# NYXFLOWER/GripNet

Measured on AMD Instinct MI355X. Metric: edges aggregated/sec, GripNet forward on pose-0, higher is better.
Workload: dtype f32

## Files before the change

### gripnet_amd/_hip.py

```python
from __future__ import annotations

import ctypes as C
import operator
import os
import threading

import torch

from ._cache import MISS, VersionedCache

_LIB_PATH = os.environ.get("GN_HIP_LIBRARY") or os.path.join(os.path.dirname(os.path.abspath(__file__)), "lib",
                                                            "libgripnet_hip.so")
_lib = None
_lock = threading.Lock()

GN_OK, GN_ERR_INVALID_ARG, GN_ERR_HIP, GN_ERR_INDEX_RANGE, GN_ERR_UNSUPPORTED, GN_ERR_EDGE_COUNT = range(6)
GN_RGCN_PARTIAL, GN_RGCN_ARITH_FAST, GN_RGCN_BASIS_TRANSPOSED = 1, 4, 64
GN_RGCN_PATH_SHIFT = 8
RGCN_PATHS = {"auto": 0, "pair": 1, "lds": 3, "general": 4, "table": 5}
GN_GEMM_RELU, GN_GEMM_ARITH_FAST, GN_GEMM_B_TRANSPOSED, GN_GEMM_ACCUMULATE, GN_GEMM_A_TRANSPOSED, GN_GEMM_JOIN_BATCH, GN_GEMM_OUT_BF16 = 1, 2, 4, 8, 16, 32, 64
GN_DM_TYPES_SORTED = 1
GN_DM_TYPE_TASKS = 2
ABI_VERSION = 162

_p, _i64, _int, _sz = C.c_void_p, C.c_int64, C.c_int, C.c_size_t

SIGNATURES = {
    "gn_version": (_int, []),
    "gn_last_error": (C.c_char_p, []),
    "gn_time_next_launch": (_int, [_p, _p]),
    "gn_host_scratch_release": (_sz, []),
    "gn_device_blocks_live": (_i64, []),
    "gn_time_launch_pending": (_int, []),
    "gn_gcn_plan_create": (_int, [_p, _p, _p, _i64, _i64, _int, _p, C.POINTER(_p)]),
    "gn_bipartite_plan_create": (_int, [_p, _p, _p, _i64, _i64, _i64, _p, C.POINTER(_p)]),
    "gn_sum_plan_create": (_int, [_p, _p, _p, _i64, _i64, _i64, _p, C.POINTER(_p)]),
    "gn_graph_plan_destroy": (None, [_p]),
    "gn_graph_plan_input_edges": (_i64, [_p]),
    "gn_graph_plan_nnz": (_i64, [_p]),
    "gn_graph_plan_export": (_int, [_p, _p, _p, _p]),
    "gn_graph_aggregate_f32": (_int, [_p, _p, _i64, _i64, _p, _i64, _p, _int, _p, _i64, _p, _p, _p]),
    "gn_split_planes_bytes": (_sz, [_i64, _int]),
    "gn_split_planes_f32": (_int, [_p, _i64, _i64, _i64, _i64, _p, _p]),
    "gn_transform_fusable": (_int, [_i64, _i64]),
    "gn_graph_transform_fusable": (_int, [_p, _i64, _i64]),
    "gn_graph_plan_build_blocked": (_int, [_p, _i64, _p]),
    "gn_graph_plan_blocked_cols": (_i64, [_p]),
    "gn_graph_blocked_applicable": (_int, [_p, _p, _i64, _i64, _p, _i64, _p, _p, _i64]),
    "gn_graph_chain_applicable": (_int, [_p, _p, _p, _i64, _i64, _p, _i64, _p, _p, _i64, _p]),
    "gn_graph_aggregate_chain_f32": (_int, [_p, _p, _p, _i64, _i64, _p, _i64, _p, _int, _p, _i64, _p, _p]),
    "gn_graph_gather_chained_f32": (_int, [_p, _p, _i64, _p]),
    "gn_graph_aggregate_tail_f32": (_int, [_p, _p, _i64, _i64, _p, _i64, _p, _int, _p, _i64, _p, _p, _p, _p, _int, _p]),
    "gn_graph_plan_build_transpose": (_int, [_p, _p]),
    "gn_graph_aggregate_t_f32": (_int, [_p, _p, _i64, _i64, _p, _i64, _p]),
    "gn_xtg_wide_supported": (_int, [_i64, _i64, _i64]),
    "gn_gemm_f32": (_int, [_p, _i64, _i64, _p, _i64, _p, _i64, _i64, _p, _i64, _i64, _i64, _i64, _i64, _i64, _p, _int, _p]),
    "gn_gemm_addend_f32": (_int, [_p, _i64, _i64, _p, _i64, _p, _i64, _i64, _p, _i64, _i64, _i64, _i64, _i64, _i64, _p, _p, _i64, _int, _p]),
    "gn_merge_f32": (_int, [_p, _i64, _p, _i64, _p, _i64, _i64, _i64, _int, _p]),
    "gn_softmax_rows_f32": (_int, [_p, _i64, _i64, _i64, _p]),
    "gn_softmax_rows_backward_f32": (_int, [_p, _i64, _p, _i64, _p, _i64, _i64, _i64, _p]),
    "gn_class_scores_f32": (_int, [_p, _i64, _i64, _p, _i64, _p, _i64, _i64, _i64, _int, _p, _i64, _p]),
    "gn_rgcn_plan_create": (_int, [_p, _p, _p, _int, _i64, _i64, _i64, _i64, _i64, _p, C.POINTER(_p)]),
    "gn_rgcn_plan_create_ex": (_int, [_p, _p, _p, _int, _i64, _i64, _i64, _i64, _i64, _int, _p, C.POINTER(_p)]),
    "gn_rgcn_plan_destroy": (None, [_p]),
    "gn_rgcn_plan_input_edges": (_i64, [_p]),
    "gn_rgcn_workspace_bytes": (_sz, [_p, _i64, _i64, _i64, _int]),
    "gn_rgcn_forward_path": (_int, [_p, _i64, _i64, _i64, _int]),
    "gn_rgcn_forward_choice": (_int, [_p, _p, _i64, _i64, _i64, _i64, _int, C.POINTER(_sz)]),
    "gn_cast_bf16": (_int, [_p, _i64, _p, _i64, _i64, _i64, _p]),
    "gn_graph_aggregate_bf16": (_int, [_p, _p, _i64, _i64, _p, _int, _p, _i64, _p, _p]),
    "gn_rgcn_forward_f32": (_int, [_p, _p, _i64, _i64, _p, _p, _i64, _p, _p, _i64, _int, _int, _p, _i64, _p, _p, _p, _sz, _p]),
    "gn_rgcn_finalize_f32": (_int, [_p, _p, _i64, _p, _i64, _i64, _p, _p, _i64, _int, _p, _i64, _p, _p]),
    "gn_distmult_forward_f32": (_int, [_p, _i64, _i64, _i64, _p, _p, _p, _p, _i64, _i64, _i64, _int, _p, _p, _p]),
    "gn_distmult_packed_forward_f32": (_int, [_p, _i64, _i64, _i64, _p, _p, _p, _i64, _i64, _i64, _int, _p, _p, _p]),
    "gn_distmult_plan_create": (_int, [_p, _p, _p, _i64, _i64, _i64, _i64, _p, C.POINTER(_p)]),
    "gn_distmult_plan_destroy": (None, [_p]),
    "gn_distmult_plan_edges": (_i64, [_p]),
    "gn_distmult_plan_forward_f32": (_int, [_p, _p, _i64, _i64, _p, _i64, _int, _p, _p]),
    "gn_distmult_plan_forward_cols_f32": (_int, [_p, _p, _i64, _i64, _i64, _i64, _p, _i64, _int, _p, _p]),
    "gn_xtg_workspace_bytes": (_sz, [_i64, _i64]),
# ... 223 lines not shown
    def __init__(self):
        self.calls, self.keep = [], []

    def __enter__(self):
        global _recorder
        self._prev, _recorder = _recorder, self
        return self

    def __exit__(self, *exc):
        global _recorder
        _recorder = self._prev


_recorder = None


def replay(calls):
    t = _timer
    for fn, args, name, tag in calls:
        if t is not None and (t.only is None or name in t.only):
            seen = t._seen.get(name, 0)
            t._seen[name] = seen + 1
            if seen % t.every == 0:
                status = _timed_call(t, fn, args, name, tag)
                if status:
                    check(status)
                continue
        status = fn(*args)
        if status:
            check(status)


_ENV_HOOKS = ("GN_DISABLE_FAST", "GN_DISABLE_QUAD", "GN_DISABLE_BLOCKED", "GN_BLOCKED_ANY", "GN_DISABLE_LDS_TABLE",
              "GN_ENABLE_CHAIN")
_ENV_NEUTRAL = ("GN_PLAN_THREADS", "GN_SAMPLER_TASKS", "GN_RGCN_SLAB_MB")
_ENV_DATA = getattr(os.environ, "_data", None)
_ENV_KEYS = tuple(k.encode() for k in _ENV_HOOKS) if isinstance(_ENV_DATA, dict) and all(isinstance(k, bytes) for k in list(_ENV_DATA)[:1]) else None


def release_host_scratch() -> int:
    return int(load().gn_host_scratch_release())


def device_blocks_live() -> int:
    return int(load().gn_device_blocks_live())


def env_stamp():
    if _ENV_KEYS is not None:
        d = _ENV_DATA
        return tuple([d.get(k) for k in _ENV_KEYS])
    return tuple([os.environ.get(k) for k in _ENV_HOOKS])


def launch_context(device):
    index = device.index
    return torch.cuda.current_device(), (_raw_stream(index) if _raw_stream is not None else torch.cuda.current_stream(index).cuda_stream)


class CallMemo:

    DEPTH = 8

    def __init__(self):
        self.entries = {}
        self.last = None

# ... 257 lines not shown
        require_gpu(edge_index, edge_weight)
        ei, src, dst, e = edge_rows(edge_index)
        w = None if edge_weight is None else edge_weight.to(torch.float32).contiguous()
        if w is not None and w.numel() != e:
            raise ValueError("edge_weight has {} entries for {} edges".format(w.numel(), e))
        plan = cls(None, ei.device, kind)
        plan._create(create, ei.device, src, dst, ptr(w), e, int(size_a), int(size_b))
        plan.n_rows, plan.n_table = int(n_rows), int(n_table)
        return plan

    @classmethod
    def gcn(cls, edge_index, num_nodes, edge_weight=None, improved=False):
        return cls._build("gcn", "gn_gcn_plan_create", edge_index, edge_weight, num_nodes, num_nodes, num_nodes, bool(improved))

    @classmethod
    def bipartite(cls, edge_index, num_sources, num_targets, edge_weight=None):
        return cls._build("bipartite", "gn_bipartite_plan_create", edge_index, edge_weight, num_sources, num_targets,
                          num_sources, num_targets)

    @classmethod
    def plain_sum(cls, edge_index, num_sources, num_targets):
        return cls._build("sum", "gn_sum_plan_create", edge_index, None, num_sources, num_targets, num_sources, num_targets)

    def build_blocked(self, cols: int):
        if self.kind == "gcn" and cols <= 32:
            with torch.cuda.device(self.device):
                check(load().gn_graph_plan_build_blocked(self._h, 16 if cols <= 16 else 32, stream_ptr(self.device)))
        return self.blocked_cols

    @property
    def blocked_cols(self) -> int:
        return int(load().gn_graph_plan_blocked_cols(self._h))

    def blocked_ok(self, x: torch.Tensor, weight: torch.Tensor, bias, out: torch.Tensor) -> bool:
        return bool(load().gn_graph_blocked_applicable(self._h, x.data_ptr(), ld(x), x.shape[1], weight.data_ptr(), weight.shape[1],
                                                       None if bias is None else bias.data_ptr(), out.data_ptr(), ld(out)))

    def transform_ok(self, fin: int, fout: int, x: torch.Tensor) -> bool:
        return (bool(load().gn_graph_transform_fusable(self._h, int(fin), int(fout))) and ld(x) % 4 == 0
                and x.data_ptr() % 16 == 0)

    @property
    def input_edges(self) -> int:
        return int(load().gn_graph_plan_input_edges(self._h))

    @property
    def nnz(self) -> int:
        return int(load().gn_graph_plan_nnz(self._h))

    def export(self):
        if self._export is None:
            n = self.nnz
            ei = torch.empty((2, n), dtype=torch.int64, device=self.device)
            nrm = torch.empty((n,), dtype=torch.float32, device=self.device)
            check(load().gn_graph_plan_export(self._h, ptr(ei), ptr(nrm), stream_ptr(self.device)))
            self._export = (ei, nrm)
        return self._export

    def __iter__(self):
        return iter(self.export())

    def aggregate(self, xw: torch.Tensor, bias, relu: bool, out: torch.Tensor, side=None, weight=None, planes=None, tail=None):
        sc = side_copy(side)
        pd = None
        if planes is not None:
            pd = planes[0].desc(planes[1], planes[2])
# ... 653 lines not shown
```

### gripnet_amd/csrc/common.h

```cpp
#pragma once

#include <hip/hip_runtime.h>
#include <hip/hip_ext.h>

#include <algorithm>
#include <atomic>
#include <cstdarg>
#include <cstdint>
#include <cstdio>
#include <cstdlib>
#include <cstring>
#include <memory>
#include <thread>
#include <type_traits>
#include <vector>

#include "gripnet_hip.h"
#include "host_parallel.hpp"

namespace gn {

constexpr int kWave = 64;

inline char* error_buffer() {
// ... 166 lines not shown

struct LaunchEvents { hipEvent_t start = nullptr, stop = nullptr; };
LaunchEvents take_launch_events();

}

struct gn_graph_plan {
    int64_t input_edges = 0;
    int64_t nnz = 0;
    int64_t rows = 0;
    int64_t table_rows = 0;
    int64_t max_row_nnz = 0;
    int is_gcn = 0;
    gn::DevBuf<int32_t> rowptr;
    gn::DevBuf<int32_t> col;
    gn::DevBuf<float> coef;
    gn::DevBuf<int64_t> ref_edge_index;
    gn::DevBuf<float> ref_norm;
    int ell_ok = 0;
    gn::DevBuf<uint32_t> ell_col;
    gn::DevBuf<float> ell_coef;
    int has_transpose = 0;
    gn::DevBuf<int32_t> t_rowptr;
    gn::DevBuf<int32_t> t_col;
    gn::DevBuf<float> t_coef;
    gn::DevBuf<float> dis;
    int unit_weights = 0;
    int plain_ones = 0;
    int blk_ok = 0, blk_cols = 0;
    int blk_cw = 0;
    int blk_rows = 0;
    int blk_cells = 0;
    int64_t blk_iters = 0;
    gn::DevBuf<float> blk_dis;
    gn::DevBuf<int32_t> blk_tile_off;
    gn::DevBuf<int32_t> blk_tile_rows;
    gn::DevBuf<float> blk_tile_dis;
    gn::DevBuf<uint32_t> blk_ids;
    gn::DevBuf<int32_t> blk_cell;
    gn::DevBuf<float> blk_table;
};

struct gn_rgcn_plan {
    int64_t input_edges = 0;
    int64_t edge_lo = 0, edge_hi = 0;
    int64_t shard_edges = 0;
    int64_t num_nodes = 0;
    int64_t num_relations = 0;
    int64_t max_row_nnz = 0;
    gn::DevBuf<float> indeg;
    gn::DevBuf<int32_t> rowptr;
    gn::DevBuf<uint32_t> key;
    gn::DevBuf<int32_t> row_order;
    int64_t heavy_rows = 0;
    gn::DevBuf<int32_t> dw_items;
    int64_t n_dw_items = 0, n_dw_parts = 0;
    gn::DevBuf<int32_t> dw_multi;
    int64_t n_dw_multi = 0;
    gn::DevBuf<int32_t> seg_begin;
    gn::DevBuf<uint32_t> packed;
    gn::DevBuf<int32_t> wg_begin;
    gn::DevBuf<int32_t> wg_items;
    int fast_groups = 0, fast_ts = 0;
    size_t fast_lds_bytes = 0;
    int fast_cols = 32;
    int fast_ok = 0;
// ... 17 lines not shown
```

### gripnet_amd/csrc/distmult_quad.cuh

```cuda
#pragma once

#include "common.h"

namespace gn_dm {

constexpr int kMaxPhases = 8;
#ifndef GN_DM_THREADS
#define GN_DM_THREADS 1024
#endif
constexpr int kThreads = GN_DM_THREADS;
constexpr size_t kLdsBudget = 150 * 1024;

typedef float f32x2 __attribute__((ext_vector_type(2)));
typedef float f32x4 __attribute__((ext_vector_type(4)));


template <int CTRL>
__device__ __forceinline__ int dpp_i(int x) { return __builtin_amdgcn_mov_dpp(x, CTRL, 0xf, 0xf, true); }
template <int CTRL>
__device__ __forceinline__ float dpp_add(float x) {
    return x + __builtin_bit_cast(float, __builtin_amdgcn_update_dpp(0, __builtin_bit_cast(int, x), CTRL, 0xf, 0xf, false));
}
__device__ __forceinline__ float row_sum16(float x) {
    x = dpp_add<0xB1>(x);
    x = dpp_add<0x4E>(x);
    x = dpp_add<0x141>(x);
    x = dpp_add<0x140>(x);
    return x;
}

__device__ __forceinline__ float sigmoid_f32(float x) { return __builtin_amdgcn_rcpf(1.0f + __expf(-x)); }

template <int W4>
__device__ __forceinline__ void fill_table(float4* lds4, const float* __restrict__ z, int64_t ld_z, int n, int c0, int w4rt,
                                           int stride4, int tid) {
    const int w4 = W4 > 0 ? W4 : w4rt;
    const int total = n * w4;
    const int rot = (int)((blockIdx.x * 977u) % (unsigned)total);
    for (int base = 0; base < total; base += 8 * kThreads) {
        float4 v[8];
        int at[8];
#pragma unroll
        for (int k = 0; k < 8; ++k) {
            int i = min(base + k * kThreads + tid, total - 1) + rot;
            i = i < total ? i : i - total;
            const int row = i / w4, c4 = i - row * w4;
            at[k] = row * stride4 + c4;
            v[k] = *reinterpret_cast<const float4*>(z + (int64_t)row * ld_z + c0 + 4 * c4);
        }
#pragma unroll
        for (int k = 0; k < 8; ++k)
            if (base + k * kThreads + tid < total) lds4[at[k]] = v[k];
    }
    const int pad = stride4 - w4;
    for (int i = tid; i < n * pad; i += kThreads) {
// ... 71 lines not shown
```

### gripnet_amd/csrc/gcn_blocked.hip

```cpp
#include "aggregate.cuh"
#include "layout_blocked.hpp"

#include <algorithm>
#include <numeric>
#include <vector>

namespace {

typedef float f32x4 __attribute__((ext_vector_type(4)));
typedef uint32_t u32x2 __attribute__((ext_vector_type(2)));
typedef float f32x2 __attribute__((ext_vector_type(2)));

#ifndef GN_COL_THREADS
#define GN_COL_THREADS 1024
#endif
constexpr int kColThreads = GN_COL_THREADS;
constexpr int kColWaves = kColThreads / 64;
static_assert(kColWaves == gn_layout::kColLayoutWaves, "the plan cuts a range's tiles into the waves of one workgroup");
constexpr size_t kColLdsBytes = 160 * 1024;
constexpr int kColSlack = gn_layout::kColLayoutSlack;
constexpr int kWaveInts = 12;

bool blocked_disabled() {
    if (gn::fast_paths_disabled()) return true;
    const char* e = getenv("GN_DISABLE_BLOCKED");
    return e && e[0] == '1';
}

struct TransArgs {
    const float* x; int64_t ld_x;
    const float* w;
    const float* dis;
    float* table;
// ... 57 lines not shown
        for (int nt = 0; nt < NT; ++nt) {
            const f32x4 v = real ? acc[nt] * scale : (f32x4){0.f, 0.f, 0.f, 0.f};
            if constexpr (CW == 2) {
                float* o = a.table + ((size_t)(8 * nt + 2 * j) * a.rows_pad + row) * 2;
                *reinterpret_cast<f32x2*>(o) = (f32x2){v[0], v[1]};
                *reinterpret_cast<f32x2*>(o + (size_t)a.rows_pad * 2) = (f32x2){v[2], v[3]};
            } else {
                float* o = a.table + (size_t)(16 * nt + 4 * j) * a.rows_pad + row;
#pragma unroll
                for (int c = 0; c < 4; ++c) o[(size_t)c * a.rows_pad] = v[c];
            }
        }
    }
}

struct ColArgs {
    const float* table;
    const int32_t* cell;
    const int32_t* tile_off;
    const int32_t* tile_rows;
    const float* tile_dis;
    const u32x2* ids;
    const float* dis; const float* bias;
    float* out; int64_t ld_out;
    int n, rows_pad, groups, ranges, relu;
    gn_side_copy side;
    float* next_table;
};

#ifdef GN_STAMPS
__device__ unsigned long long g_blk_stamps[2][512][4];
#endif

template <int CW, bool NEXT>
__device__ __forceinline__ void col_gather(const ColArgs& a, int stamp_set) {
    typedef float vec_t __attribute__((ext_vector_type(CW)));
    extern __shared__ f32x4 lds4[];
    const int tid = threadIdx.x, lane = tid & 63;
    const int wave = __builtin_amdgcn_readfirstlane(tid >> 6);
    const int q = lane >> 2, j = lane & 3;
    const int wg = blockIdx.x, per_x = (a.ranges + 7) / 8;
    const int x = wg & 7, k = wg >> 3;
    const int range = x * per_x + k / a.groups, cg = k % a.groups;
    const bool live = range < a.ranges;
#ifdef GN_STAMPS
    const unsigned long long st0 = __builtin_amdgcn_s_memrealtime();
#endif
    const int32_t* __restrict__ cell = a.cell + ((size_t)(live ? range : 0) * kColWaves + wave) * kWaveInts;
    const int c0 = cell[0], c1 = cell[1];
    int it = cell[2];
    const int it_last = cell[3];
    const int e0 = cell[4], e1 = cell[5], e2 = cell[6], e3 = cell[7], e4 = cell[8];
    if (live) {
        const int total = a.rows_pad * CW / 4;
        const f32x4* __restrict__ src = reinterpret_cast<const f32x4*>(a.table + (size_t)cg * a.rows_pad * CW);
        for (int i = wave * 64; i < total; i += kColThreads)
            __builtin_amdgcn_global_load_lds((const __attribute__((address_space(1))) void*)(src + i + lane),
                                             (__attribute__((address_space(3))) void*)(lds4 + i), 16, 0, 0);
    }
    do {
    if (!live) break;
    asm volatile("" ::: "memory");
    int tile_end = e0;
    const u32x2* __restrict__ sp = a.ids + (size_t)it * 64 + lane;
    u32x2 wa[8], wb[8];
#pragma unroll
    for (int k = 0; k < 8; ++k) wa[k] = sp[64 * k];
#pragma unroll
    for (int k = 0; k < 8; ++k) wb[k] = sp[512 + 64 * k];
    sp += 1024;
    const int32_t* __restrict__ trp = a.tile_rows + (size_t)c0 * 16 + q;
    const float* __restrict__ tdp = a.tile_dis + (size_t)c0 * 16 + q;
    int row = trp[0];
    const int row1 = trp[16], row2 = trp[32], row3 = trp[48];
    float d = tdp[0];
    const float d1 = tdp[16], d2 = tdp[32], d3 = tdp[48];
    int t = c0;
    vec_t bias = (vec_t)(0.f);
    if (a.bias) bias = *reinterpret_cast<const vec_t*>(a.bias + CW * cg);
    asm volatile("s_waitcnt vmcnt(0)" ::: "memory");
    __syncthreads();
#ifdef GN_STAMPS
    const unsigned long long st1 = __builtin_amdgcn_s_memrealtime();
#endif
    const vec_t* __restrict__ tab = reinterpret_cast<const vec_t*>(lds4);
    vec_t acc = (vec_t)(0.f);
#define GN_COL_FLUSH()                                                                                         \
    do {                                                                                                       \
        _Pragma("unroll") for (int c = 0; c < CW; ++c) {                                                       \
            float v = acc[c];                                                                                  \
            v += __shfl_xor(v, 1);                                                                             \
            v += __shfl_xor(v, 2);                                                                             \
            acc[c] = v;                                                                                        \
        }                                                                                                      \
        if (j == 0 && row >= 0) {                                                                              \
            vec_t r = acc * d + bias;                                                                          \
            if (a.relu) {                                                                                      \
                _Pragma("unroll") for (int c = 0; c < CW; ++c) r[c] = fmaxf(r[c], 0.f);                        \
            }                                                                                                  \
            *reinterpret_cast<vec_t*>(a.out + (int64_t)row * a.ld_out + CW * cg) = r;                          \
            if constexpr (NEXT)                                                                                \
                *reinterpret_cast<vec_t*>(a.next_table + ((size_t)cg * a.rows_pad + row) * CW) = r * d;        \
        }                                                                                                      \
        acc = (vec_t)(0.f);                                                                                    \
        ++t;                                                                                                   \
        const int kk = t - c0;                                                                                 \
        tile_end = kk == 1 ? e1 : (kk == 2 ? e2 : (kk == 3 ? e3 : (kk == 4 ? e4 : a.tile_off[t + 1])));       \
        if (kk < 4) {                                                                                          \
            row = kk == 1 ? row1 : (kk == 2 ? row2 : row3);                                                    \
            d = kk == 1 ? d1 : (kk == 2 ? d2 : d3);                                                            \
        } else {                                                                                               \
            row = a.tile_rows[(size_t)t * 16 + q];                                                             \
            d = a.tile_dis[(size_t)t * 16 + q];                                                                \
        }                                                                                                      \
    } while (0)
#define GN_COL_CONSUME(w)                                                                                      \
    _Pragma("unroll") for (int k = 0; k < 8; ++k) {                                                            \
        while (t < c1 && it == tile_end) GN_COL_FLUSH();                                                       \
        if (it < it_last) {                                                                                    \
            const uint32_t s0 = w[k].x & 0xffffu, s1 = w[k].x >> 16, s2 = w[k].y & 0xffffu, s3 = w[k].y >> 16; \
            acc += (tab[s0] + tab[s1]) + (tab[s2] + tab[s3]);                                                  \
            ++it;                                                                                              \
        }                                                                                                      \
    }
    while (it < it_last) {
        GN_COL_CONSUME(wa)
        if (it >= it_last) break;
#pragma unroll
        for (int k = 0; k < 8; ++k) wa[k] = sp[64 * k];
        GN_COL_CONSUME(wb)
#pragma unroll
        for (int k = 0; k < 8; ++k) wb[k] = sp[512 + 64 * k];
        sp += 1024;
    }
    while (t < c1) GN_COL_FLUSH();
#undef GN_COL_CONSUME
#undef GN_COL_FLUSH
#ifdef GN_STAMPS
    if (tid == 0 && blockIdx.x < 512) {
        unsigned long long* o = g_blk_stamps[stamp_set & 1][blockIdx.x];
        o[0] = st0; o[1] = st1; o[2] = __builtin_amdgcn_s_memrealtime(); o[3] = 0;
    }
#endif
    } while (0);
    gn::side_copy_stream(a.side, blockIdx.x * (int64_t)blockDim.x + threadIdx.x, (int64_t)gridDim.x * blockDim.x);
}

template <int CW>
__global__ __launch_bounds__(kColThreads) void k_col_gather(ColArgs a, int stamp_set) { col_gather<CW, false>(a, stamp_set); }
template <int CW>
__global__ __launch_bounds__(kColThreads) void k_col_gather_next(ColArgs a, int stamp_set) { col_gather<CW, true>(a, stamp_set); }

template <int FIN, int NT>
void launch_transform(const TransArgs& t, int cw, hipStream_t st) {
    const int grid = (int)std::min<int64_t>(gn::ceil_div(t.rows_pad / 16, 4), GN_AGG_GRID);
    if (cw == 2) k_col_transform<FIN, NT, 2><<<grid, 256, 0, st>>>(t); else k_col_transform<FIN, NT, 1><<<grid, 256, 0, st>>>(t);
}

}

bool gn_blocked_applicable(const gn_graph_plan* plan, const float* x, int64_t ld_x, int64_t fin, const float* w, int64_t fout,
                           const float* bias, const float* out, int64_t ld_out) {
    if (!plan->blk_ok || blocked_disabled()) return false;
    const int cw = plan->blk_cw;
    if ((ld_out % cw) != 0 || (reinterpret_cast<uintptr_t>(out) % (4 * cw)) != 0 ||
        (bias && (reinterpret_cast<uintptr_t>(bias) % (4 * cw)) != 0)) return false;
    if (!(fout == 16 || fout == 32) || fout > plan->blk_cols) return false;
    if (w) {
        if (!(fin == 16 || fin == 32 || fin == 64)) return false;
        if (!gn::aligned16(w)) return false;
    } else if (fin != fout) {
        return false;
    }
    return (ld_x % 4) == 0 && gn::aligned16(x);
}

namespace {

gn_status blocked_transform(const gn_graph_plan* plan, const float* x, int64_t ld_x, int64_t fin, const float* w, int64_t fout,
                            hipStream_t st) {
    TransArgs t;
    t.x = x; t.ld_x = ld_x; t.w = w; t.dis = plan->blk_dis.p; t.table = plan->blk_table.p; t.n = (int)plan->rows;
    t.rows_pad = plan->blk_rows;
    const int cw = plan->blk_cw;
    switch ((int)((w ? fin : fout) * 100 + fout)) {
        case 1616: launch_transform<16, 1>(t, cw, st); break;
        case 3216: launch_transform<32, 1>(t, cw, st); break;
        case 6416: launch_transform<64, 1>(t, cw, st); break;
        case 1632: launch_transform<16, 2>(t, cw, st); break;
        case 3232: launch_transform<32, 2>(t, cw, st); break;
        case 6432: launch_transform<64, 2>(t, cw, st); break;
        default: return gn::fail(GN_ERR_UNSUPPORTED, "no LDS-staged kernel for %lld -> %lld features", (long long)fin, (long long)fout);
    }
    GN_LAUNCH_CHECK();
    return GN_OK;
}

gn_status blocked_gather(const gn_graph_plan* plan, int64_t fout, const float* bias, int relu, float* out, int64_t ld_out,
                         const gn_side_copy& side, float* next_table, int stamp_set, hipStream_t st) {
    const int cw = plan->blk_cw;
    GN_REQUIRE((ld_out % cw) == 0 && (reinterpret_cast<uintptr_t>(out) % (4 * cw)) == 0 &&
               (!bias || (reinterpret_cast<uintptr_t>(bias) % (4 * cw)) == 0),
               "the LDS-staged path writes %d-float column groups: out and bias must be aligned to them", cw);
    ColArgs a;
    a.table = plan->blk_table.p; a.cell = plan->blk_cell.p; a.tile_off = plan->blk_tile_off.p; a.tile_rows = plan->blk_tile_rows.p;
    a.tile_dis = plan->blk_tile_dis.p;
    a.ids = reinterpret_cast<const u32x2*>(plan->blk_ids.p); a.dis = plan->blk_dis.p; a.bias = bias;
    a.out = out; a.ld_out = ld_out; a.n = (int)plan->rows; a.rows_pad = plan->blk_rows;
    a.groups = (int)(fout / cw); a.ranges = plan->blk_cells; a.relu = relu; a.side = side; a.next_table = next_table;
    const int per_x = (a.ranges + 7) / 8;
    const int grid = 8 * per_x * a.groups;
    const size_t lds = (size_t)plan->blk_rows * cw * sizeof(float);
    auto launch = [&](auto kernel) {
        gn_status s = gn::allow_large_lds(reinterpret_cast<const void*>(kernel), (int)kColLdsBytes);
        if (s == GN_OK) kernel<<<grid, kColThreads, lds, st>>>(a, stamp_set);
        return s;
    };
    gn_status s;
    if (next_table) s = cw == 2 ? launch(k_col_gather_next<2>) : launch(k_col_gather_next<1>);
    else s = cw == 2 ? launch(k_col_gather<2>) : launch(k_col_gather<1>);
    if (s != GN_OK) return s;
    GN_LAUNCH_CHECK();
    return GN_OK;
}

bool chain_disabled() {
    const char* e = getenv("GN_ENABLE_CHAIN");
    return !(e && e[0] == '1') || blocked_disabled();
}

bool chain_plans_match(const gn_graph_plan* plan, const gn_graph_plan* next) {
    return plan && next && plan != next && plan->blk_ok && next->blk_ok && plan->is_gcn && next->is_gcn && plan->unit_weights &&
           next->unit_weights && plan->rows == next->rows && plan->nnz == next->nnz && plan->blk_rows == next->blk_rows &&
           plan->blk_cw == next->blk_cw && plan->blk_cells == next->blk_cells && plan->blk_iters == next->blk_iters &&
           next->blk_cols >= 16;
}

}

gn_status gn_blocked_aggregate(const gn_graph_plan* plan, const float* x, int64_t ld_x, int64_t fin, const float* w,
                               int64_t fout, const float* bias, int relu, float* out, int64_t ld_out,
                               const gn_side_copy& side, hipStream_t st) {
    const gn_status s = blocked_transform(plan, x, ld_x, fin, w, fout, st);
    return s != GN_OK ? s : blocked_gather(plan, fout, bias, relu, out, ld_out, side, nullptr, fin == 32 ? 0 : 1, st);
}

extern "C" int gn_graph_chain_applicable(const gn_graph_plan* plan, const gn_graph_plan* next, const float* x, int64_t ld_x,
                                         int64_t num_features, const float* weight, int64_t out_features, const float* bias,
                                         const float* out, int64_t ld_out, const float* out_next) {
    if (chain_disabled() || !chain_plans_match(plan, next) || !weight || out_features != 16) return 0;
    if (!gn_blocked_applicable(plan, x, ld_x, num_features, weight, out_features, bias, out, ld_out)) return 0;
    return (reinterpret_cast<uintptr_t>(out_next) % (4 * next->blk_cw)) == 0 ? 1 : 0;
}
// ... 46 lines not shown
        rows_pad = gn::ceil_div((N + 1) * cw * 4, 1024) * 1024 / (cw * 4);
        if (rows_pad * cw * 4 > (int64_t)kColLdsBytes) return GN_OK;
    }
    const int groups = (int)(cols / cw);
    const int R = std::max(1, std::min<int>(256 / groups, (int)gn::ceil_div(N, 64)));

    GN_LAP(nullptr);
    gn::ArenaHold arena;
    std::vector<int32_t> rp(N + 1), col(nnz);
    GN_HIP(hipMemcpyAsync(rp.data(), plan->rowptr.p, (N + 1) * sizeof(int32_t), hipMemcpyDeviceToHost, st));
    GN_HIP(hipMemcpyAsync(col.data(), plan->col.p, nnz * sizeof(int32_t), hipMemcpyDeviceToHost, st));
    std::vector<float> dis_host((size_t)rows_pad + 16, 0.f);
    GN_HIP(hipMemcpyAsync(dis_host.data(), plan->dis.p, N * sizeof(float), hipMemcpyDeviceToHost, st));
    GN_HIP(hipStreamSynchronize(st));

    GN_LAP("blocked: CSR to the host");
    gn_layout::BlockedLayout bl = gn_layout::build_blocked_layout(N, R, rp, col, dis_host);
    GN_LAP("blocked: host schedule");
    if (bl.failed) return gn::fail(GN_ERR_UNSUPPORTED, "internal: an edge was not scheduled");
    if (!bl.ok) return GN_OK;
    plan->blk_ok = 0;
    GN_HIP(plan->blk_dis.upload(dis_host, st));
    GN_HIP(plan->blk_tile_off.upload(bl.tile_off, st));
    GN_HIP(plan->blk_tile_rows.upload(bl.tile_rows, st));
    GN_HIP(plan->blk_tile_dis.upload(bl.tile_dis, st));
    GN_HIP(plan->blk_ids.upload(bl.ids.data(), bl.ids.size() / 2, st));
    GN_HIP(plan->blk_cell.upload(bl.cell, st));
    GN_HIP(plan->blk_table.alloc((size_t)rows_pad * cols));
    GN_HIP(hipMemsetAsync(plan->blk_table.p, 0, (size_t)rows_pad * cols * sizeof(float), st));
    GN_HIP(hipStreamSynchronize(st));
    GN_LAP("blocked: upload");
    plan->blk_cols = (int)cols; plan->blk_cw = cw; plan->blk_rows = (int)rows_pad; plan->blk_cells = R;
    plan->blk_iters = bl.iters_total;
    plan->blk_ok = 1;
    return GN_OK;
}

#ifdef GN_STAMPS
extern "C" __attribute__((visibility("default"))) int gn_debug_read_blk_stamps(unsigned long long* host_out) {
    return (int)hipMemcpyFromSymbol(host_out, HIP_SYMBOL(g_blk_stamps), sizeof(unsigned long long) * 2 * 512 * 4);
}
#endif

extern "C" int64_t gn_graph_plan_blocked_cols(const gn_graph_plan* plan) {
    return (plan && plan->blk_ok && !blocked_disabled()) ? plan->blk_cols : 0;
}
```

### include/gripnet_hip.h

```cpp
#ifndef GRIPNET_HIP_H
#define GRIPNET_HIP_H

#include <stddef.h>
#include <stdint.h>

#ifdef __cplusplus
extern "C" {
#endif

#define GN_VERSION 162

#if defined(GN_BUILDING)
#define GN_API __attribute__((visibility("default")))
#else
#define GN_API
#endif

typedef enum gn_status {
    GN_OK = 0,
    GN_ERR_INVALID_ARG = 1,
    GN_ERR_HIP = 2,
    GN_ERR_INDEX_RANGE = 3,
    GN_ERR_UNSUPPORTED = 4,
    GN_ERR_EDGE_COUNT = 5
} gn_status;

typedef struct gn_side_copy {
    const float* src; int64_t ld_src;
    float* dst; int64_t ld_dst;
    int64_t rows, cols;
    int mode;
} gn_side_copy;

typedef struct gn_split_planes {
    void* planes;
    int64_t rows;
    int nt;
    int col_main;
    int col_side;
} gn_split_planes;

typedef struct gn_graph_plan gn_graph_plan;
typedef struct gn_rgcn_plan gn_rgcn_plan;

GN_API int gn_version(void);
GN_API const char* gn_last_error(void);
GN_API int64_t gn_device_blocks_live(void);

GN_API gn_status gn_gcn_plan_create(const int64_t* src, const int64_t* dst, const float* w, int64_t num_edges,
                             int64_t num_nodes, int improved, void* stream, gn_graph_plan** plan);

GN_API gn_status gn_bipartite_plan_create(const int64_t* src, const int64_t* dst, const float* w, int64_t num_edges,
                                   int64_t num_sources, int64_t num_targets, void* stream, gn_graph_plan** plan);

GN_API gn_status gn_sum_plan_create(const int64_t* src, const int64_t* dst, const float* w, int64_t num_edges,
                             int64_t num_sources, int64_t num_targets, void* stream, gn_graph_plan** plan);

GN_API void gn_graph_plan_destroy(gn_graph_plan* plan);
GN_API int64_t gn_graph_plan_input_edges(const gn_graph_plan* plan);
GN_API int64_t gn_graph_plan_nnz(const gn_graph_plan* plan);
GN_API gn_status gn_graph_plan_export(const gn_graph_plan* plan, int64_t* edge_index_out, float* norm_out, void* stream);

GN_API gn_status gn_graph_aggregate_f32(const gn_graph_plan* plan, const float* xw, int64_t ld_xw, int64_t num_features,
                                 const float* weight , int64_t out_features,
                                 const float* bias, int relu, float* out, int64_t ld_out,
                                 const gn_side_copy* side , const gn_split_planes* planes ,
                                 void* stream);
GN_API size_t gn_split_planes_bytes(int64_t rows, int nt);
GN_API gn_status gn_split_planes_f32(const float* src, int64_t ld_src, int64_t rows, int64_t cols, int64_t col0,
                              const gn_split_planes* planes, void* stream);
GN_API int gn_transform_fusable(int64_t in_features, int64_t out_features);
GN_API int gn_graph_transform_fusable(const gn_graph_plan* plan, int64_t in_features, int64_t out_features);

GN_API gn_status gn_graph_plan_build_blocked(gn_graph_plan* plan, int64_t cols, void* stream);
GN_API int64_t gn_graph_plan_blocked_cols(const gn_graph_plan* plan);
GN_API int gn_graph_blocked_applicable(const gn_graph_plan* plan, const float* x, int64_t ld_x, int64_t num_features,
                                       const float* weight, int64_t out_features, const float* bias, const float* out,
                                       int64_t ld_out);

GN_API int gn_graph_chain_applicable(const gn_graph_plan* plan, const gn_graph_plan* next, const float* x, int64_t ld_x,
                                     int64_t num_features, const float* weight, int64_t out_features, const float* bias,
                                     const float* out, int64_t ld_out, const float* out_next);
GN_API gn_status gn_graph_aggregate_chain_f32(const gn_graph_plan* plan, const gn_graph_plan* next, const float* x, int64_t ld_x,
                                       int64_t num_features, const float* weight, int64_t out_features, const float* bias,
                                       int relu, float* out, int64_t ld_out, const gn_side_copy* side ,
                                       void* stream);
GN_API gn_status gn_graph_gather_chained_f32(const gn_graph_plan* plan, float* out, int64_t ld_out, void* stream);
GN_API gn_status gn_graph_aggregate_tail_f32(const gn_graph_plan* plan, const float* x, int64_t ld_x, int64_t num_features,
                                      const float* weight, int64_t out_features, const float* bias, int relu, float* out,
                                      int64_t ld_out, const gn_side_copy* side ,
                                      const gn_split_planes* planes , const float* tail_w,
                                      const float* tail_b , int tail_relu, void* stream);

GN_API gn_status gn_cast_bf16(const float* src, int64_t ld_src, uint16_t* dst, int64_t ld_dst, int64_t rows, int64_t cols,
                       void* stream);
GN_API gn_status gn_graph_aggregate_bf16(const gn_graph_plan* plan, const uint16_t* table, int64_t ld_table, int64_t num_features,
                                  const float* bias, int relu, float* out, int64_t ld_out,
                                  const gn_side_copy* side , void* stream);

GN_API gn_status gn_graph_plan_build_transpose(gn_graph_plan* plan, void* stream);
GN_API gn_status gn_graph_aggregate_t_f32(const gn_graph_plan* plan, const float* g, int64_t ld_g, int64_t num_features,
                                   float* out, int64_t ld_out, void* stream);

#define GN_GEMM_RELU 1
#define GN_GEMM_ARITH_FAST 2
#define GN_GEMM_B_TRANSPOSED 4
#define GN_GEMM_ACCUMULATE 8
#define GN_GEMM_A_TRANSPOSED 16
// ... 246 lines not shown
```

Measured before the change: 63.64 billion.

## Stage blocked column-gather results in LDS and write out in a separate pass

The blocked GCN column gather now accumulates each tile's reduced sums into an LDS staging area, then runs a second pass that reads row indices and degree scales contiguously and writes scaled, biased outputs. This replaces per-tile scattered loads of row and scale values and per-flush writes inside the main loop. It also swaps the shuffle reductions for DPP adds and skips prefetches past the last iteration. The staged path is chosen when the table plus staging buffer fit in LDS, with an env override to force the direct path; extra LDS use may reduce occupancy.

Measured after the change: 65.29 billion, median of 6. 2.6% higher.

```diff
diff --git a/gripnet_amd/_hip.py b/gripnet_amd/_hip.py
--- a/gripnet_amd/_hip.py
+++ b/gripnet_amd/_hip.py
@@ -21,7 +21,7 @@
 GN_GEMM_RELU, GN_GEMM_ARITH_FAST, GN_GEMM_B_TRANSPOSED, GN_GEMM_ACCUMULATE, GN_GEMM_A_TRANSPOSED, GN_GEMM_JOIN_BATCH, GN_GEMM_OUT_BF16 = 1, 2, 4, 8, 16, 32, 64
 GN_DM_TYPES_SORTED = 1
 GN_DM_TYPE_TASKS = 2
-ABI_VERSION = 162
+ABI_VERSION = 163
 
 _p, _i64, _int, _sz = C.c_void_p, C.c_int64, C.c_int, C.c_size_t
 
@@ -46,6 +46,8 @@
     "gn_graph_transform_fusable": (_int, [_p, _i64, _i64]),
     "gn_graph_plan_build_blocked": (_int, [_p, _i64, _p]),
     "gn_graph_plan_blocked_cols": (_i64, [_p]),
+    "gn_graph_plan_blocked_gather_kernel": (_int, [_p]),
+    "gn_graph_plan_blocked_waves": (_i64, [_p, _p, _i64]),
     "gn_graph_blocked_applicable": (_int, [_p, _p, _i64, _i64, _p, _i64, _p, _p, _i64]),
     "gn_graph_chain_applicable": (_int, [_p, _p, _p, _i64, _i64, _p, _i64, _p, _p, _i64, _p]),
     "gn_graph_aggregate_chain_f32": (_int, [_p, _p, _p, _i64, _i64, _p, _i64, _p, _int, _p, _i64, _p, _p]),
@@ -335,7 +337,7 @@
 
 
 _ENV_HOOKS = ("GN_DISABLE_FAST", "GN_DISABLE_QUAD", "GN_DISABLE_BLOCKED", "GN_BLOCKED_ANY", "GN_DISABLE_LDS_TABLE",
-              "GN_ENABLE_CHAIN")
+              "GN_ENABLE_CHAIN", "GN_BLOCKED_DIRECT")
 _ENV_NEUTRAL = ("GN_PLAN_THREADS", "GN_SAMPLER_TASKS", "GN_RGCN_SLAB_MB")
 _ENV_DATA = getattr(os.environ, "_data", None)
 _ENV_KEYS = tuple(k.encode() for k in _ENV_HOOKS) if isinstance(_ENV_DATA, dict) and all(isinstance(k, bytes) for k in list(_ENV_DATA)[:1]) else None
@@ -659,6 +661,21 @@
     def blocked_cols(self) -> int:
         return int(load().gn_graph_plan_blocked_cols(self._h))
 
+    @property
+    def blocked_gather_kernel(self) -> str:
+        return ("", "staged", "direct")[int(load().gn_graph_plan_blocked_gather_kernel(self._h))]
+
+    def blocked_waves(self) -> torch.Tensor:
+        lib = load()
+        n = int(lib.gn_graph_plan_blocked_waves(self._h, None, 0))
+        cell = torch.zeros((n,), dtype=torch.int32)
+        if n and lib.gn_graph_plan_blocked_waves(self._h, cell.data_ptr(), n) != n:
+            raise GripNetHipError(GN_ERR_HIP, "gn_graph_plan_blocked_waves failed")
+        if n % (16 * 12):
+            raise GripNetHipError(GN_ERR_HIP, "gn_graph_plan_blocked_waves: {} ints are no whole number of 16 x 12 records".format(n))
+        cell = cell.view(-1, 16, 12).long()
+        return torch.stack([cell[:, :, 1] - cell[:, :, 0], cell[:, :, 3] - cell[:, :, 2]], dim=2)
+
     def blocked_ok(self, x: torch.Tensor, weight: torch.Tensor, bias, out: torch.Tensor) -> bool:
         return bool(load().gn_graph_blocked_applicable(self._h, x.data_ptr(), ld(x), x.shape[1], weight.data_ptr(), weight.shape[1],
                                                        None if bias is None else bias.data_ptr(), out.data_ptr(), ld(out)))
diff --git a/gripnet_amd/csrc/common.h b/gripnet_amd/csrc/common.h
--- a/gripnet_amd/csrc/common.h
+++ b/gripnet_amd/csrc/common.h
@@ -222,6 +222,7 @@
     int blk_rows = 0;
     int blk_cells = 0;
     int64_t blk_iters = 0;
+    int blk_range_tiles = 0;
     gn::DevBuf<float> blk_dis;
     gn::DevBuf<int32_t> blk_tile_off;
     gn::DevBuf<int32_t> blk_tile_rows;
diff --git a/gripnet_amd/csrc/distmult_quad.cuh b/gripnet_amd/csrc/distmult_quad.cuh
--- a/gripnet_amd/csrc/distmult_quad.cuh
+++ b/gripnet_amd/csrc/distmult_quad.cuh
@@ -1,6 +1,7 @@
 #pragma once
 
 #include "common.h"
+#include "dpp.cuh"
 
 namespace gn_dm {
 
@@ -15,12 +16,8 @@
 typedef float f32x4 __attribute__((ext_vector_type(4)));
 
 
-template <int CTRL>
-__device__ __forceinline__ int dpp_i(int x) { return __builtin_amdgcn_mov_dpp(x, CTRL, 0xf, 0xf, true); }
-template <int CTRL>
-__device__ __forceinline__ float dpp_add(float x) {
-    return x + __builtin_bit_cast(float, __builtin_amdgcn_update_dpp(0, __builtin_bit_cast(int, x), CTRL, 0xf, 0xf, false));
-}
+using gn::dpp_i;
+using gn::dpp_add;
 __device__ __forceinline__ float row_sum16(float x) {
     x = dpp_add<0xB1>(x);
     x = dpp_add<0x4E>(x);
diff --git a/gripnet_amd/csrc/dpp.cuh b/gripnet_amd/csrc/dpp.cuh
--- /dev/null
+++ b/gripnet_amd/csrc/dpp.cuh
@@ -0,0 +1,12 @@
+#pragma once
+
+namespace gn {
+
+template <int CTRL>
+__device__ __forceinline__ int dpp_i(int x) { return __builtin_amdgcn_mov_dpp(x, CTRL, 0xf, 0xf, true); }
+template <int CTRL>
+__device__ __forceinline__ float dpp_add(float x) {
+    return x + __builtin_bit_cast(float, __builtin_amdgcn_update_dpp(0, __builtin_bit_cast(int, x), CTRL, 0xf, 0xf, false));
+}
+
+}
diff --git a/gripnet_amd/csrc/gcn_blocked.hip b/gripnet_amd/csrc/gcn_blocked.hip
--- a/gripnet_amd/csrc/gcn_blocked.hip
+++ b/gripnet_amd/csrc/gcn_blocked.hip
@@ -1,4 +1,5 @@
 #include "aggregate.cuh"
+#include "dpp.cuh"
 #include "layout_blocked.hpp"
 
 #include <algorithm>
@@ -122,7 +123,21 @@
 __device__ unsigned long long g_blk_stamps[2][512][4];
 #endif
 
-template <int CW, bool NEXT>
+template <int CW, typename V>
+__device__ __forceinline__ V scale_bias(V acc, float d, V bias) {
+    V r;
+    if constexpr (CW == 2) {
+#pragma unroll
+        for (int c = 0; c < CW; ++c) r[c] = __builtin_fmaf(acc[c], d, bias[c]);
+    } else {
+#pragma clang fp contract(off)
+        const float p = acc[0] * d;
+        r[0] = p + bias[0];
+    }
+    return r;
+}
+
+template <int CW, bool NEXT, bool STAGED>
 __device__ __forceinline__ void col_gather(const ColArgs& a, int stamp_set) {
     typedef float vec_t __attribute__((ext_vector_type(CW)));
     extern __shared__ f32x4 lds4[];
@@ -141,6 +156,7 @@
     int it = cell[2];
     const int it_last = cell[3];
     const int e0 = cell[4], e1 = cell[5], e2 = cell[6], e3 = cell[7], e4 = cell[8];
+    const int range_c0 = a.cell[(size_t)(live ? range : 0) * kColWaves * kWaveInts];
     if (live) {
         const int total = a.rows_pad * CW / 4;
         const f32x4* __restrict__ src = reinterpret_cast<const f32x4*>(a.table + (size_t)cg * a.rows_pad * CW);
@@ -159,32 +175,33 @@
 #pragma unroll
     for (int k = 0; k < 8; ++k) wb[k] = sp[512 + 64 * k];
     sp += 1024;
-    const int32_t* __restrict__ trp = a.tile_rows + (size_t)c0 * 16 + q;
-    const float* __restrict__ tdp = a.tile_dis + (size_t)c0 * 16 + q;
-    int row = trp[0];
-    const int row1 = trp[16], row2 = trp[32], row3 = trp[48];
-    float d = tdp[0];
-    const float d1 = tdp[16], d2 = tdp[32], d3 = tdp[48];
+    int row = -1, row1 = -1, row2 = -1, row3 = -1;
+    float d = 0.f, d1 = 0.f, d2 = 0.f, d3 = 0.f;
+    vec_t bias = (vec_t)(0.f);
+    if constexpr (!STAGED) {
+        const int32_t* __restrict__ trp = a.tile_rows + (size_t)c0 * 16 + q;
+        const float* __restrict__ tdp = a.tile_dis + (size_t)c0 * 16 + q;
+        row = trp[0]; row1 = trp[16]; row2 = trp[32]; row3 = trp[48];
+        d = tdp[0]; d1 = tdp[16]; d2 = tdp[32]; d3 = tdp[48];
+        if (a.bias) bias = *reinterpret_cast<const vec_t*>(a.bias + CW * cg);
+    }
     int t = c0;
-    vec_t bias = (vec_t)(0.f);
-    if (a.bias) bias = *reinterpret_cast<const vec_t*>(a.bias + CW * cg);
     asm volatile("s_waitcnt vmcnt(0)" ::: "memory");
     __syncthreads();
 #ifdef GN_STAMPS
     const unsigned long long st1 = __builtin_amdgcn_s_memrealtime();
 #endif
     const vec_t* __restrict__ tab = reinterpret_cast<const vec_t*>(lds4);
+    vec_t* stage = reinterpret_cast<vec_t*>(lds4) + a.rows_pad;
     vec_t acc = (vec_t)(0.f);
 #define GN_COL_FLUSH()                                                                                         \
     do {                                                                                                       \
-        _Pragma("unroll") for (int c = 0; c < CW; ++c) {                                                       \
-            float v = acc[c];                                                                                  \
-            v += __shfl_xor(v, 1);                                                                             \
-            v += __shfl_xor(v, 2);                                                                             \
-            acc[c] = v;                                                                                        \
-        }                                                                                                      \
-        if (j == 0 && row >= 0) {                                                                              \
-            vec_t r = acc * d + bias;                                                                          \
+        _Pragma("unroll") for (int c = 0; c < CW; ++c)                                                         \
+            acc[c] = gn::dpp_add<0x4E>(gn::dpp_add<0xB1>(acc[c]));            \
+        if constexpr (STAGED) {                                                                                \
+            if (j == 0) stage[(t - range_c0) * 16 + q] = acc;                                                  \
+        } else if (j == 0 && row >= 0) {                                                                       \
+            vec_t r = scale_bias<CW>(acc, d, bias);                                                            \
             if (a.relu) {                                                                                      \
                 _Pragma("unroll") for (int c = 0; c < CW; ++c) r[c] = fmaxf(r[c], 0.f);                        \
             }                                                                                                  \
@@ -196,12 +213,14 @@
         ++t;                                                                                                   \
         const int kk = t - c0;                                                                                 \
         tile_end = kk == 1 ? e1 : (kk == 2 ? e2 : (kk == 3 ? e3 : (kk == 4 ? e4 : a.tile_off[t + 1])));       \
-        if (kk < 4) {                                                                                          \
-            row = kk == 1 ? row1 : (kk == 2 ? row2 : row3);                                                    \
-            d = kk == 1 ? d1 : (kk == 2 ? d2 : d3);                                                            \
-        } else {                                                                                               \
-            row = a.tile_rows[(size_t)t * 16 + q];                                                             \
-            d = a.tile_dis[(size_t)t * 16 + q];                                                                \
+        if constexpr (!STAGED) {                                                                               \
+            if (kk < 4) {                                                                                      \
+                row = kk == 1 ? row1 : (kk == 2 ? row2 : row3);                                                \
+                d = kk == 1 ? d1 : (kk == 2 ? d2 : d3);                                                        \
+            } else {                                                                                           \
+                row = a.tile_rows[(size_t)t * 16 + q];                                                         \
+                d = a.tile_dis[(size_t)t * 16 + q];                                                            \
+            }                                                                                                  \
         }                                                                                                      \
     } while (0)
 #define GN_COL_CONSUME(w)                                                                                      \
@@ -216,20 +235,53 @@
     while (it < it_last) {
         GN_COL_CONSUME(wa)
         if (it >= it_last) break;
-#pragma unroll
-        for (int k = 0; k < 8; ++k) wa[k] = sp[64 * k];
+        if (it + 8 < it_last) {
+#pragma unroll
+            for (int k = 0; k < 8; ++k) wa[k] = sp[64 * k];
+        }
         GN_COL_CONSUME(wb)
-#pragma unroll
-        for (int k = 0; k < 8; ++k) wb[k] = sp[512 + 64 * k];
+        if (it + 8 < it_last) {
+#pragma unroll
+            for (int k = 0; k < 8; ++k) wb[k] = sp[512 + 64 * k];
+        }
         sp += 1024;
     }
     while (t < c1) GN_COL_FLUSH();
 #undef GN_COL_CONSUME
 #undef GN_COL_FLUSH
 #ifdef GN_STAMPS
+    const unsigned long long st2 = __builtin_amdgcn_s_memrealtime();
+#endif
+    if constexpr (STAGED) {
+        vec_t wbias = (vec_t)(0.f);
+        if (a.bias) wbias = *reinterpret_cast<const vec_t*>(a.bias + CW * cg);
+        const int s_end = c1 * 16;
+        for (int s0 = c0 * 16 + lane; s0 < s_end; s0 += 128) {
+            const bool two = s0 + 64 < s_end;
+            const int s1 = two ? s0 + 64 : s0;
+            int rowa = a.tile_rows[s0], rowb = a.tile_rows[s1];
+            float da = a.tile_dis[s0], db = a.tile_dis[s1];
+            const vec_t va = stage[s0 - range_c0 * 16], vb = stage[s1 - range_c0 * 16];
+            asm volatile("" : "+v"(rowa), "+v"(rowb), "+v"(da), "+v"(db));
+            vec_t ra = scale_bias<CW>(va, da, wbias), rb = scale_bias<CW>(vb, db, wbias);
+            if (a.relu) {
+#pragma unroll
+                for (int c = 0; c < CW; ++c) { ra[c] = fmaxf(ra[c], 0.f); rb[c] = fmaxf(rb[c], 0.f); }
+            }
+            if (rowa >= 0) {
+                *reinterpret_cast<vec_t*>(a.out + (int64_t)rowa * a.ld_out + CW * cg) = ra;
+                if constexpr (NEXT) *reinterpret_cast<vec_t*>(a.next_table + ((size_t)cg * a.rows_pad + rowa) * CW) = ra * da;
+            }
+            if (two && rowb >= 0) {
+                *reinterpret_cast<vec_t*>(a.out + (int64_t)rowb * a.ld_out + CW * cg) = rb;
+                if constexpr (NEXT) *reinterpret_cast<vec_t*>(a.next_table + ((size_t)cg * a.rows_pad + rowb) * CW) = rb * db;
+            }
+        }
+    }
+#ifdef GN_STAMPS
     if (tid == 0 && blockIdx.x < 512) {
         unsigned long long* o = g_blk_stamps[stamp_set & 1][blockIdx.x];
-        o[0] = st0; o[1] = st1; o[2] = __builtin_amdgcn_s_memrealtime(); o[3] = 0;
+        o[0] = st0; o[1] = st1; o[2] = __builtin_amdgcn_s_memrealtime(); o[3] = st2;
     }
 #endif
     } while (0);
@@ -237,9 +289,13 @@
 }
 
 template <int CW>
-__global__ __launch_bounds__(kColThreads) void k_col_gather(ColArgs a, int stamp_set) { col_gather<CW, false>(a, stamp_set); }
+__global__ __launch_bounds__(kColThreads) void k_col_gather(ColArgs a, int stamp_set) { col_gather<CW, false, true>(a, stamp_set); }
 template <int CW>
-__global__ __launch_bounds__(kColThreads) void k_col_gather_next(ColArgs a, int stamp_set) { col_gather<CW, true>(a, stamp_set); }
+__global__ __launch_bounds__(kColThreads) void k_col_gather_next(ColArgs a, int stamp_set) { col_gather<CW, true, true>(a, stamp_set); }
+template <int CW>
+__global__ __launch_bounds__(kColThreads) void k_col_gather_direct(ColArgs a, int stamp_set) { col_gather<CW, false, false>(a, stamp_set); }
+template <int CW>
+__global__ __launch_bounds__(kColThreads) void k_col_gather_next_direct(ColArgs a, int stamp_set) { col_gather<CW, true, false>(a, stamp_set); }
 
 template <int FIN, int NT>
 void launch_transform(const TransArgs& t, int cw, hipStream_t st) {
@@ -286,6 +342,14 @@
     return GN_OK;
 }
 
+size_t stage_bytes(const gn_graph_plan* plan) { return (size_t)plan->blk_range_tiles * 16 * plan->blk_cw * sizeof(float); }
+
+bool blocked_staged(const gn_graph_plan* plan) {
+    const char* e = getenv("GN_BLOCKED_DIRECT");
+    if (e && e[0] == '1') return false;
+    return (size_t)plan->blk_rows * plan->blk_cw * sizeof(float) + stage_bytes(plan) <= kColLdsBytes;
+}
+
 gn_status blocked_gather(const gn_graph_plan* plan, int64_t fout, const float* bias, int relu, float* out, int64_t ld_out,
                          const gn_side_copy& side, float* next_table, int stamp_set, hipStream_t st) {
     const int cw = plan->blk_cw;
@@ -300,15 +364,21 @@
     a.groups = (int)(fout / cw); a.ranges = plan->blk_cells; a.relu = relu; a.side = side; a.next_table = next_table;
     const int per_x = (a.ranges + 7) / 8;
     const int grid = 8 * per_x * a.groups;
-    const size_t lds = (size_t)plan->blk_rows * cw * sizeof(float);
+    const bool staged = blocked_staged(plan);
+    const size_t lds = (size_t)plan->blk_rows * cw * sizeof(float) + (staged ? stage_bytes(plan) : 0);
     auto launch = [&](auto kernel) {
         gn_status s = gn::allow_large_lds(reinterpret_cast<const void*>(kernel), (int)kColLdsBytes);
         if (s == GN_OK) kernel<<<grid, kColThreads, lds, st>>>(a, stamp_set);
         return s;
     };
     gn_status s;
-    if (next_table) s = cw == 2 ? launch(k_col_gather_next<2>) : launch(k_col_gather_next<1>);
-    else s = cw == 2 ? launch(k_col_gather<2>) : launch(k_col_gather<1>);
+    if (staged) {
+        if (next_table) s = cw == 2 ? launch(k_col_gather_next<2>) : launch(k_col_gather_next<1>);
+        else s = cw == 2 ? launch(k_col_gather<2>) : launch(k_col_gather<1>);
+    } else {
+        if (next_table) s = cw == 2 ? launch(k_col_gather_next_direct<2>) : launch(k_col_gather_next_direct<1>);
+        else s = cw == 2 ? launch(k_col_gather_direct<2>) : launch(k_col_gather_direct<1>);
+    }
     if (s != GN_OK) return s;
     GN_LAUNCH_CHECK();
     return GN_OK;
@@ -421,6 +491,11 @@
     GN_LAP("blocked: upload");
     plan->blk_cols = (int)cols; plan->blk_cw = cw; plan->blk_rows = (int)rows_pad; plan->blk_cells = R;
     plan->blk_iters = bl.iters_total;
+    plan->blk_range_tiles = 0;
+    for (int r = 0; r < R; ++r) {
+        const int32_t* c = bl.cell.data() + (size_t)r * kColWaves * kWaveInts;
+        plan->blk_range_tiles = std::max<int>(plan->blk_range_tiles, c[(kColWaves - 1) * kWaveInts + 1] - c[0]);
+    }
     plan->blk_ok = 1;
     return GN_OK;
 }
@@ -431,6 +506,21 @@
 }
 #endif
 
+extern "C" int gn_graph_plan_blocked_gather_kernel(const gn_graph_plan* plan) {
+    if (!plan || !plan->blk_ok || blocked_disabled()) return 0;
+    return blocked_staged(plan) ? 1 : 2;
+}
+
+extern "C" int64_t gn_graph_plan_blocked_waves(const gn_graph_plan* plan, int32_t* host_out, int64_t capacity) {
+    if (!plan || !plan->blk_ok) return 0;
+    const int64_t count = (int64_t)plan->blk_cell.n;
+    if (host_out) {
+        if (capacity < count) return -1;
+        if (hipMemcpy(host_out, plan->blk_cell.p, (size_t)count * sizeof(int32_t), hipMemcpyDeviceToHost) != hipSuccess) return -1;
+    }
+    return count;
+}
+
 extern "C" int64_t gn_graph_plan_blocked_cols(const gn_graph_plan* plan) {
     return (plan && plan->blk_ok && !blocked_disabled()) ? plan->blk_cols : 0;
 }
diff --git a/include/gripnet_hip.h b/include/gripnet_hip.h
--- a/include/gripnet_hip.h
+++ b/include/gripnet_hip.h
@@ -8,7 +8,7 @@
 extern "C" {
 #endif
 
-#define GN_VERSION 162
+#define GN_VERSION 163
 
 #if defined(GN_BUILDING)
 #define GN_API __attribute__((visibility("default")))
@@ -74,6 +74,8 @@
 
 GN_API gn_status gn_graph_plan_build_blocked(gn_graph_plan* plan, int64_t cols, void* stream);
 GN_API int64_t gn_graph_plan_blocked_cols(const gn_graph_plan* plan);
+GN_API int gn_graph_plan_blocked_gather_kernel(const gn_graph_plan* plan);
+GN_API int64_t gn_graph_plan_blocked_waves(const gn_graph_plan* plan, int32_t* host_out, int64_t capacity);
 GN_API int gn_graph_blocked_applicable(const gn_graph_plan* plan, const float* x, int64_t ld_x, int64_t num_features,
                                        const float* weight, int64_t out_features, const float* bias, const float* out,
                                        int64_t ld_out);
```
